# Duy1230/Map-Reduced-Approach-for-Vietnamese-Long-Document-Summarization

Hardware: AMD Instinct MI355X
Metric: map-phase chunks/sec (2k-tok chunk, 256-tok summary) at 1/2/4/8 MI355X (higher is better)
Workload: dtype f16

## Files before the change

map-reduced-approach-for-vietnamese-long-document-summarization_amd/csrc/gemv_common.h:

```cpp
#pragma once
#include "kernels.h"

namespace ms {

__device__ __forceinline__ uint4 ldg16(const void* p) { return *(const uint4*)p; }

__device__ __forceinline__ uint4 ldw16(const void* p) { return *(const uint4*)p; }

__host__ __device__ constexpr int vmcnt_imm(int n) { return (n & 0xF) | ((n >> 4) << 14) | (0x7 << 4) | (0xF << 8); }

__device__ __forceinline__ void lds_sync() {
  __builtin_amdgcn_fence(__ATOMIC_RELEASE, "workgroup", "local");
  __builtin_amdgcn_s_barrier();
  __builtin_amdgcn_fence(__ATOMIC_ACQUIRE, "workgroup", "local");
}

__host__ __device__ inline size_t gemv_x_lds_bytes(int M, int K) {
  return ((size_t)M * K * 2 + 1023) / 1024 * 1024;
}
__device__ __forceinline__ int x_lds(int r, int k, int K) { return r * 2 * K + (((k >> 3) ^ (r & 7)) << 4); }

__device__ __forceinline__ void gemv_dma_x(char* smem, const f16_t* __restrict__ X, int M, int K, int ldx) {
  const int kch = K >> 3, n = M * kch, lane = threadIdx.x & 63, nw = blockDim.x >> 6;
  for (int p = threadIdx.x >> 6; p * 64 < n; p += nw) {
    const int P = min(p * 64 + lane, n - 1);
    const int r = P / kch, c = P - r * kch;
    __builtin_amdgcn_global_load_lds((const void*)(X + (size_t)r * ldx + ((c ^ (r & 7)) << 3)),
                                     (LDS_AS void*)(smem + (size_t)p * 1024), 16, 0, 0);
  }
}

__host__ __device__ inline size_t gemv_xw_lds_bytes(int M, int K) { return (size_t)((M + 7) >> 3) * K * 16; }
__device__ __forceinline__ int xw_swz(int r) {
  const int t = r >> 1;
  return ((((t >> 1) ^ (t >> 2)) & 1) << 2) | ((t & 1) << 1) | ((t >> 2) & 1);
}
__device__ __forceinline__ int xw_lds(int r, int u, int c, int mp) {
  return (u * mp * 8 + r) * 128 + ((c ^ xw_swz(r)) << 4);
}
template <int U>
__device__ __forceinline__ void gemv_dma_x_wave(char* smem, const f16_t* __restrict__ X, int M, int ldx,
                                                int kbeg) {
  const int lane = threadIdx.x & 63, wave = threadIdx.x >> 6, mp = (M + 7) >> 3;
  char* base = smem + (size_t)wave * U * mp * 1024;
#pragma unroll 1
  for (int j = 0; j < mp; ++j) {
    const int r = j * 8 + (lane >> 3);
    const f16_t* src = X + (size_t)min(r, M - 1) * ldx + kbeg + (((lane & 7) ^ xw_swz(r)) << 3);
#pragma unroll
    for (int u = 0; u < U; ++u)
      __builtin_amdgcn_global_load_lds((const void*)(src + u * 64), (LDS_AS void*)(base + (size_t)(u * mp + j) * 1024),
                                       16, 0, 0);
  }
}

enum { kXGlobal = 0, kXLds = 1, kXRegs = 2, kXWave = 3 };

constexpr int kRsStage = 4096;
__host__ __device__ inline int rs_stage_floats(const RowScale& rs, int M) {
  const int n = rs.tiles * M;
  return (rs.ssq && n <= kRsStage) ? (n + 63) / 64 * 64 : 0;
}
__host__ __device__ inline size_t gemv_rinv_offset(size_t main_bytes) { return (main_bytes + 15) / 16 * 16; }
__host__ __device__ inline size_t gemv_lds_total(size_t main_bytes, const RowScale& rs, int M) {
  return gemv_rinv_offset(main_bytes) + 64 * 4 + (size_t)rs_stage_floats(rs, M) * 4;
}
template <bool HOLD>
__device__ __forceinline__ float rs_begin(char* smem, size_t rinv_off, const RowScale& rs, int M) {
  const int lane = threadIdx.x & 63, wave = threadIdx.x >> 6, nw = blockDim.x >> 6;
  if constexpr (HOLD)
    if (rs.tiles == 1) return (wave == 0 && lane < M) ? rs.ssq[lane] : 0.f;
  const int nf = rs_stage_floats(rs, M), n = rs.tiles * M;
  float* stage = (float*)(smem + rinv_off) + 64;
  for (int p = wave; p * 64 < nf; p += nw)
    __builtin_amdgcn_global_load_lds((const void*)(rs.ssq + min(p * 64 + lane, n - 1)),
                                     (LDS_AS void*)(stage + p * 64), 4, 0, 0);
  return 0.f;
}
template <bool HOLD>
__device__ __forceinline__ void rs_finish(const char* smem, size_t rinv_off, const RowScale& rs, int M,
                                          float direct) {
  const int lane = threadIdx.x & 63, wave = threadIdx.x >> 6, nw = blockDim.x >> 6;
  float* rinv = (float*)(smem + rinv_off);
  if (HOLD && rs.tiles == 1) {
    if (wave == 0 && lane < M) rinv[lane] = rs_rinv(direct, rs);
    return;
  }
  const float* stage = rinv + 64;
  for (int row = wave; row < M; row += nw) {
    float sum = 0.f;
    for (int t = lane; t < ((rs.tiles + 63) & ~63); t += 64) sum += t < rs.tiles ? stage[t * M + row] : 0.f;
    sum = wave_sum(sum);
    if (lane == 0) rinv[row] = rs_rinv(sum, rs);
  }
}

template <int EPI> constexpr bool gemv_rs_epi() {
  return EPI == MS_GEMV_EPI_STORE_F16 || EPI == MS_GEMV_EPI_SWIGLU || EPI == MS_GEMV_EPI_STORE_F32 ||
         EPI == MS_GEMV_EPI_ROPE_KV;
}

constexpr int kXRegsMaxFrags = 4;
enum { kGxLds = 0, kGxRegs = 1, kGxF32 = 2, kGxResid = 3, kGxBoth = 4 };
inline int gemv_x_mode() {
  static const int v = [] {
    const char* e = getenv("MS_GEMV_X");
    if (!e) return kGxLds;
    const char c = e[0];
    return c == 'r' && e[1] == 'e' && e[2] == 'g' ? kGxRegs : c == 'f' ? kGxF32 : c == 'r' ? kGxResid
         : c == 'b' ? kGxBoth : kGxLds;
  }();
  return v;
}
inline bool gemv_x_regs_for(int epi) {
  const int m = gemv_x_mode();
  const bool f32 = epi == MS_GEMV_EPI_STORE_F32, resid = epi == MS_GEMV_EPI_RESID_SSQ;
  return m == kGxRegs || ((m == kGxF32 || m == kGxBoth) && f32) || ((m == kGxResid || m == kGxBoth) && resid);
}
inline int qgemv_x_mode() {
  static const int v = [] {
    const char* e = getenv("MS_QGEMV_X");
    if (!e) return 2;
    return e[0] == 'r' ? 0 : e[0] == 'l' ? 1 : e[0] == 'g' ? 2 : e[0] == 's' ? 3 : 2;
  }();
  return v;
}

__device__ __forceinline__ void amax_merge_dev(float& v, int& i, float v2, int i2) {
  if (v2 > v || (v2 == v && i2 < i)) { v = v2; i = i2; }
}

struct ResidPre {
  float x, g;
};
template <int MT, int NT, int EPI, bool RS>
__device__ __forceinline__ void gemv_epilogue(const float* red, const float* rinv, int M, int N, int ldo,
                                              void* __restrict__ out, int n0, const GemvArgs& ga,
                                              const ResidPre& pre);
__device__ __forceinline__ void gemv_elem(int e, int NT, int n0, int& row, int& col, int& c) {
  const int mn = e >> 8, l = (e >> 2) & 63, j = e & 3;
  row = (mn / NT) * 16 + 4 * (l >> 4) + j;
  c = l & 15;
  col = n0 + (mn % NT) * 16 + c;
}
template <int EPI, bool RAW = false>
__device__ __forceinline__ ResidPre resid_prefetch(int M, int N, int ldo, const void* out, int n0,
                                                   const GemvArgs& ga) {
  ResidPre p{0.f, 0.f};
  if constexpr (EPI == MS_GEMV_EPI_RESID_SSQ) {
    const int rtv = ga.rt > 0 ? ga.rt : 16;
    if ((int)threadIdx.x < 256) {
      int row, col, c;
      gemv_elem(threadIdx.x, 1, n0, row, col, c);
      if (row < M && c < rtv && col < N) {
        p.x = ((const float*)out)[(size_t)row * ldo + col];
        if (ga.xg_out) p.g = RAW ? __uint_as_float((unsigned)ga.gamma[col]) : h2f(ga.gamma[col]);
      }
    }
  }
  return p;
// ... 143 lines not shown
```

map-reduced-approach-for-vietnamese-long-document-summarization_amd/csrc/k_gemv.hip:

```cpp
#include "gemv_common.h"

namespace ms {

struct GemvPlan {
  int MT, NT, waves, U, tiles;
};

static GemvPlan gemv_plan(int M, int N, int K, int epi, int force_waves = 0, int rt = 0) {
  GemvPlan p;
  p.MT = (M + 15) / 16;
  p.NT = (epi == MS_GEMV_EPI_SWIGLU) ? 2 : 1;
  const int rows = p.NT == 1 && rt > 0 ? rt : 16 * p.NT;
  p.tiles = (N + rows - 1) / rows;
  const int steps = K / 64;
  int best_w = 0;
  if (force_waves > 0 && steps % force_waves == 0 && steps / force_waves <= 8) {
    best_w = force_waves;
  } else {
    for (int w = 16; w >= 1; --w)
      if (steps % w == 0 && steps / w <= 8) { best_w = w; break; }
  }
  p.waves = best_w;
  p.U = best_w ? steps / best_w : 0;
  return p;
}

size_t gemv_workspace_bytes(int, int, int) { return 256; }

constexpr size_t kMaxLds = 160 * 1024;

static size_t gemv_lds_main(const GemvPlan& p, int M, int K, int xm) {
  size_t xs = xm == kXLds ? gemv_x_lds_bytes(M, K) : xm == kXWave ? gemv_xw_lds_bytes(M, K) : 0;
  const size_t red = (size_t)p.waves * p.MT * p.NT * 256 * 4;
  return xs > red ? xs : red;
}
static size_t gemv_lds_bytes(const GemvPlan& p, int M, int K, int xm, const RowScale& rs = RowScale{}) {
  return gemv_lds_total(gemv_lds_main(p, M, K, xm), rs, M);
}

constexpr int kGvStampBlocks = 1024, kGvStamps = 32;
__device__ unsigned long long g_gemv_stamps[kGvStampBlocks * kGvStamps];
#define GV_STAMP(k)                                     \
  do {                                                  \
    if constexpr (STAMP) {                              \
      __builtin_amdgcn_sched_barrier(0);                \
      ts[k] = __builtin_amdgcn_s_memrealtime();         \
      __builtin_amdgcn_sched_barrier(0);                \
    }                                                   \
  } while (0)

template <int MT, int NT, int EPI, int U, int XM, bool RS, bool WF, bool STAMP>
__device__ __forceinline__ void gemv_body(const f16_t* __restrict__ X, const f16_t* __restrict__ W,
                                          void* __restrict__ out, int M, int N, int K, int ldk, int ldo,
                                          int rinv_off, const GemvArgs& ga) {
  static_assert(!WF || XM == kXLds || XM == kXWave, "weight-first applies to the DMA-staged forms");
  static_assert(XM != kXWave || WF, "per-wave slices come with the weight-first order");
  extern __shared__ __attribute__((aligned(16))) char smem[];
  const int tid = threadIdx.x, lane = tid & 63, wave = tid >> 6;
  const int fr = lane & 15, fg = lane >> 4;
  unsigned long long ts[STAMP ? 12 : 1] = {};
  GV_STAMP(0);
  const int rt = NT == 1 && ga.rt > 0 ? ga.rt : 16;
  const int n0 = blockIdx.x * (NT == 1 ? rt : 16 * NT);
  const int kbeg = wave * U * 64;
  if constexpr (EPI == MS_GEMV_EPI_STORE_F32) {
    X += (size_t)blockIdx.y * K;
    W += (size_t)blockIdx.y * K;
    out = (float*)out + (size_t)blockIdx.y * (ga.slab_rows > 0 ? ga.slab_rows : M) * ldo;
  }
  constexpr bool kXL = XM == kXLds || XM == kXWave;
  constexpr bool kRsEarly = kXL && NT == 1;
  constexpr bool kBar = XM == kXLds || (RS && NT == 1);
  constexpr int kAfterX = WF ? (U - 1) * NT * 2 : U * NT * 2;

  uint4 w[U][NT][2];
  if constexpr (WF) {
#pragma unroll
    for (int n = 0; n < NT; ++n) {
      const int wrow = NT == 1 ? n0 + min(fr, rt - 1) : n0 + n * 16 + fr;
      const f16_t* wp = W + (size_t)min(wrow, N - 1) * ldk + kbeg + 16 * fg;
      w[0][n][0] = ldw16(wp);
      w[0][n][1] = ldw16(wp + 8);
    }
    GV_STAMP(2);
    __builtin_amdgcn_sched_barrier(0);
  }
  if constexpr (RS) rs_begin<false>(smem, rinv_off, ga.rs, M);
  ResidPre pre = resid_prefetch<EPI, WF>(M, N, ldo, out, n0, ga);
  if constexpr (XM == kXLds) gemv_dma_x(smem, X, M, K, ldk);
  if constexpr (XM == kXWave) gemv_dma_x_wave<U>(smem, X, M, ldk, kbeg);
  uint4 xr[XM == kXRegs ? U : 1][XM == kXRegs ? MT : 1][2];
  if constexpr (XM == kXRegs) {
#pragma unroll
    for (int u = 0; u < U; ++u)
#pragma unroll
      for (int m = 0; m < MT; ++m) {
        const f16_t* xg = X + (size_t)min(m * 16 + fr, M - 1) * ldk + kbeg + u * 64 + 16 * fg;
        xr[u][m][0] = ldg16(xg);
        xr[u][m][1] = ldg16(xg + 8);
      }
  }
  GV_STAMP(3);
  __builtin_amdgcn_sched_barrier(0);
  if constexpr (WF) {
#pragma unroll
    for (int u = 1; u < U; ++u)
#pragma unroll
      for (int n = 0; n < NT; ++n) {
        const int wrow = NT == 1 ? n0 + min(fr, rt - 1) : n0 + n * 16 + fr;
        const f16_t* wp = W + (size_t)min(wrow, N - 1) * ldk + kbeg + 16 * fg;
        w[u][n][0] = ldw16(wp + u * 64);
        w[u][n][1] = ldw16(wp + u * 64 + 8);
      }
  } else {
#pragma unroll
    for (int n = 0; n < NT; ++n) {
      const int wrow = NT == 1 ? n0 + min(fr, rt - 1) : n0 + n * 16 + fr;
      const f16_t* wp = W + (size_t)min(wrow, N - 1) * ldk + kbeg + 16 * fg;
#pragma unroll
      for (int u = 0; u < U; ++u) {
        w[u][n][0] = ldw16(wp + u * 64);
        w[u][n][1] = ldw16(wp + u * 64 + 8);
        if (n == 0 && u == 0) GV_STAMP(2);
      }
    }
  }
  GV_STAMP(4);
  if constexpr (kXL) {
    __builtin_amdgcn_sched_barrier(0);
    __builtin_amdgcn_s_waitcnt(vmcnt_imm(kAfterX));
    GV_STAMP(5);
    if constexpr (kBar) __builtin_amdgcn_s_barrier();
    GV_STAMP(6);
    if constexpr (RS && NT == 1) rs_finish<false>(smem, rinv_off, ga.rs, M, 0.f);
  }

  f32x4 acc[MT][NT];
#pragma unroll
  for (int m = 0; m < MT; ++m)
#pragma unroll
    for (int n = 0; n < NT; ++n) acc[m][n] = f32x4{0.f, 0.f, 0.f, 0.f};
  const int mp = (M + 7) >> 3;
  const char* xw = smem + (size_t)wave * U * mp * 1024;
#pragma unroll
  for (int u = 0; u < U; ++u) {
    if constexpr (STAMP) {
      if (u == 0) {
        __builtin_amdgcn_s_waitcnt(vmcnt_imm(WF ? (U - 1) * NT * 2 : (U - 1) * 2));
        GV_STAMP(7);
      }
      if (u == U - 1) {
        __builtin_amdgcn_s_waitcnt(vmcnt_imm(0));
        GV_STAMP(8);
      }
    }
#pragma unroll
    for (int m = 0; m < MT; ++m) {
      const int xrow = min(m * 16 + fr, M - 1);
      f16x8 x0, x1;
      if constexpr (XM == kXRegs) {
        x0 = as_f16x8(xr[u][m][0]);
        x1 = as_f16x8(xr[u][m][1]);
      } else if constexpr (XM == kXLds) {
        const int k0 = kbeg + u * 64 + 16 * fg;
        x0 = *(const f16x8*)(smem + x_lds(xrow, k0, K));
        x1 = *(const f16x8*)(smem + x_lds(xrow, k0 + 8, K));
      } else if constexpr (XM == kXWave) {
        x0 = *(const f16x8*)(xw + xw_lds(xrow, u, 2 * fg, mp));
        x1 = *(const f16x8*)(xw + xw_lds(xrow, u, 2 * fg + 1, mp));
      } else {
        const f16_t* xg = X + (size_t)xrow * ldk + kbeg + u * 64 + 16 * fg;
        x0 = as_f16x8(ldg16(xg));
        x1 = as_f16x8(ldg16(xg + 8));
      }
#pragma unroll
      for (int n = 0; n < NT; ++n) {
        acc[m][n] = mfma16(x0, as_f16x8(w[u][n][0]), acc[m][n]);
        acc[m][n] = mfma16(x1, as_f16x8(w[u][n][1]), acc[m][n]);
      }
    }
  }
  if constexpr (WF && EPI == MS_GEMV_EPI_RESID_SSQ) resid_gain(pre);
  GV_STAMP(9);
  unsigned long long* t_red = nullptr;
  if constexpr (STAMP) t_red = &ts[10];
  gemv_finish<MT, NT, EPI, RS, kRsEarly, false>(acc, smem, rinv_off, M, N, ldo, out, n0, ga, pre, 0.f, t_red);
  if constexpr (STAMP) {
    GV_STAMP(11);
    const int nw = blockDim.x >> 6, blk = blockIdx.y * gridDim.x + blockIdx.x;
    if (lane == 0 && (wave == 0 || wave == nw - 1) && blk < kGvStampBlocks) {
      unsigned hw, xcc;
      asm volatile("s_getreg_b32 %0, hwreg(HW_REG_HW_ID)" : "=s"(hw));
      asm volatile("s_getreg_b32 %0, hwreg(HW_REG_XCC_ID)" : "=s"(xcc));
      ts[1] = ((unsigned long long)xcc << 32) | hw;
      unsigned long long* dst = g_gemv_stamps + (size_t)blk * kGvStamps + (wave == 0 ? 0 : 16);
#pragma unroll
      for (int k = 0; k < 12; ++k) dst[k] = ts[k];
    }
  }
}

template <int MT, int NT, int EPI, int U, int XM, bool RS>
__global__ __launch_bounds__(1024) void gemv_kernel(const f16_t* __restrict__ X,
                                                    const f16_t* __restrict__ W,
                                                    void* __restrict__ out, int M, int N, int K,
                                                    int ldk, int ldo, int rinv_off, GemvArgs ga) {
  extern __shared__ __attribute__((aligned(16))) char smem[];
  const int tid = threadIdx.x, lane = tid & 63, wave = tid >> 6;
  const int fr = lane & 15, fg = lane >> 4;
  const int rt = NT == 1 && ga.rt > 0 ? ga.rt : 16;
  const int n0 = blockIdx.x * (NT == 1 ? rt : 16 * NT);
  const int kbeg = wave * U * 64;
  if constexpr (EPI == MS_GEMV_EPI_STORE_F32) {
    X += (size_t)blockIdx.y * K;
    W += (size_t)blockIdx.y * K;
    out = (float*)out + (size_t)blockIdx.y * (ga.slab_rows > 0 ? ga.slab_rows : M) * ldo;
  }

  constexpr bool kRsEarly = XM == kXLds && NT == 1;
  if constexpr (RS) rs_begin<false>(smem, rinv_off, ga.rs, M);
  const ResidPre pre = resid_prefetch<EPI>(M, N, ldo, out, n0, ga);
  if constexpr (XM == kXLds) gemv_dma_x(smem, X, M, K, ldk);
  uint4 xr[XM == kXRegs ? U : 1][XM == kXRegs ? MT : 1][2];
  if constexpr (XM == kXRegs) {
#pragma unroll
    for (int u = 0; u < U; ++u)
#pragma unroll
      for (int m = 0; m < MT; ++m) {
        const f16_t* xg = X + (size_t)min(m * 16 + fr, M - 1) * ldk + kbeg + u * 64 + 16 * fg;
        xr[u][m][0] = ldg16(xg);
        xr[u][m][1] = ldg16(xg + 8);
      }
  }
  __builtin_amdgcn_sched_barrier(0);
  uint4 w[U][NT][2];
#pragma unroll
  for (int n = 0; n < NT; ++n) {
    const int wrow = NT == 1 ? n0 + min(fr, rt - 1) : n0 + n * 16 + fr;
    const f16_t* wp = W + (size_t)min(wrow, N - 1) * ldk + kbeg + 16 * fg;
#pragma unroll
    for (int u = 0; u < U; ++u) {
      w[u][n][0] = ldw16(wp + u * 64);
      w[u][n][1] = ldw16(wp + u * 64 + 8);
    }
  }
  if constexpr (XM == kXLds) {
    __builtin_amdgcn_sched_barrier(0);
    __builtin_amdgcn_s_waitcnt(vmcnt_imm(U * NT * 2));
    __builtin_amdgcn_s_barrier();
    if constexpr (RS && NT == 1) rs_finish<false>(smem, rinv_off, ga.rs, M, 0.f);
  }

  f32x4 acc[MT][NT];
#pragma unroll
  for (int m = 0; m < MT; ++m)
#pragma unroll
    for (int n = 0; n < NT; ++n) acc[m][n] = f32x4{0.f, 0.f, 0.f, 0.f};
#pragma unroll
  for (int u = 0; u < U; ++u) {
#pragma unroll
    for (int m = 0; m < MT; ++m) {
      const int xrow = min(m * 16 + fr, M - 1);
      f16x8 x0, x1;
      if constexpr (XM == kXRegs) {
        x0 = as_f16x8(xr[u][m][0]);
        x1 = as_f16x8(xr[u][m][1]);
      } else if constexpr (XM == kXLds) {
        const int k0 = kbeg + u * 64 + 16 * fg;
        x0 = *(const f16x8*)(smem + x_lds(xrow, k0, K));
        x1 = *(const f16x8*)(smem + x_lds(xrow, k0 + 8, K));
      } else {
        const f16_t* xg = X + (size_t)xrow * ldk + kbeg + u * 64 + 16 * fg;
        x0 = as_f16x8(ldg16(xg));
        x1 = as_f16x8(ldg16(xg + 8));
      }
#pragma unroll
      for (int n = 0; n < NT; ++n) {
        acc[m][n] = mfma16(x0, as_f16x8(w[u][n][0]), acc[m][n]);
        acc[m][n] = mfma16(x1, as_f16x8(w[u][n][1]), acc[m][n]);
      }
    }
  }
  gemv_finish<MT, NT, EPI, RS, kRsEarly, false>(acc, smem, rinv_off, M, N, ldo, out, n0, ga, pre);
}

template <int MT, int NT, int EPI, int U, int XM, bool RS>
__global__ __launch_bounds__(1024) void gemv_wf_kernel(const f16_t* __restrict__ X,
                                                       const f16_t* __restrict__ W,
                                                       void* __restrict__ out, int M, int N, int K,
                                                       int ldk, int ldo, int rinv_off, GemvArgs ga) {
  gemv_body<MT, NT, EPI, U, XM, RS, true, false>(X, W, out, M, N, K, ldk, ldo, rinv_off, ga);
}

template <int NT, int EPI, int U, int XM, bool RS, bool WF>
__global__ __launch_bounds__(1024) void gemv_stamp_kernel(const f16_t* __restrict__ X,
                                                          const f16_t* __restrict__ W,
                                                          void* __restrict__ out, int M, int N, int K,
                                                          int ldk, int ldo, int rinv_off, GemvArgs ga) {
  gemv_body<1, NT, EPI, U, XM, RS, WF, true>(X, W, out, M, N, K, ldk, ldo, rinv_off, ga);
}

void gemv_stamps(unsigned long long* host, int n) {
  n = std::min(n, kGvStampBlocks * kGvStamps);
  (void)hipMemcpyFromSymbol(host, HIP_SYMBOL(g_gemv_stamps), (size_t)n * sizeof(unsigned long long));
  void* p = nullptr;
  if (hipGetSymbolAddress(&p, HIP_SYMBOL(g_gemv_stamps)) == hipSuccess)
    (void)hipMemset(p, 0, sizeof(unsigned long long) * kGvStampBlocks * kGvStamps);
}

static bool gemv_stamps_on() {
  static const bool on = [] { const char* e = getenv("MS_GEMV_STAMPS"); return e && atoi(e); }();
  return on;
}

enum { kGcQkv = 0, kGcO, kGcGateUp, kGcDown, kGcLmHead, kGcCount };
static int g_gemv_class_order[kGcCount] = {0, 2, 1, 2, 0};
static int g_gemv_order = [] {
  const char* e = getenv("MS_GEMV_ORDER");
  if (!e || !e[0]) return -1;
  auto dig = [](char c) { return c >= '0' && c <= '2' ? c - '0' : 0; };
  if (!e[1]) return dig(e[0]);
  for (int i = 0; i < kGcCount && e[i]; ++i) g_gemv_class_order[i] = dig(e[i]);
  return -1;
}();
void set_gemv_order(int v) { g_gemv_order = v; }
static int gemv_order_for(int epi, int N, int U) {
  if (g_gemv_order >= 0) return g_gemv_order;
  if (epi == MS_GEMV_EPI_SWIGLU) return g_gemv_class_order[kGcGateUp];
  if (epi == MS_GEMV_EPI_RESID_SSQ) return g_gemv_class_order[U <= 4 ? kGcO : kGcDown];
  if (epi == MS_GEMV_EPI_ARGMAX || (epi == MS_GEMV_EPI_STORE_F32 && N >= 65536)) return g_gemv_class_order[kGcLmHead];
  if (epi == MS_GEMV_EPI_STORE_F32) return g_gemv_class_order[kGcQkv];
  return 0;
}

template <int MT, int NT, int EPI, int U, bool RS>
static void gemv_go_rs(const f16_t* X, const f16_t* W, void* out, int M, int N, int K, int ldk,
                       const dim3& grid, const dim3& blk, size_t lds, int ro, int ldo, int xm, int ord,
                       const GemvArgs& ga, hipStream_t s) {
#define GL(...) MS_LAUNCH((__VA_ARGS__), grid, blk, lds, s, X, W, out, M, N, K, ldk, ldo, ro, ga)
  if constexpr (MT * U <= kXRegsMaxFrags) {
    if (xm == kXRegs) {
      GL(gemv_kernel<MT, NT, EPI, U, kXRegs, RS>);
      return;
    }
  }
  constexpr bool kStampEpi = EPI == MS_GEMV_EPI_STORE_F32 || EPI == MS_GEMV_EPI_SWIGLU ||
                             EPI == MS_GEMV_EPI_RESID_SSQ || EPI == MS_GEMV_EPI_ARGMAX;
  if constexpr (MT == 1 && (U == 1 || U == 3 || U == 8) && kStampEpi) {
    if (gemv_stamps_on() && (xm == kXLds || xm == kXWave)) {
      if (xm == kXWave) GL(gemv_stamp_kernel<NT, EPI, U, kXWave, RS, true>);
      else if (ord) GL(gemv_stamp_kernel<NT, EPI, U, kXLds, RS, true>);
      else GL(gemv_stamp_kernel<NT, EPI, U, kXLds, RS, false>);
      return;
    }
  }
  if (xm == kXWave) GL(gemv_wf_kernel<MT, NT, EPI, U, kXWave, RS>);
  else if (xm == kXLds && ord) GL(gemv_wf_kernel<MT, NT, EPI, U, kXLds, RS>);
  else if (xm == kXLds) GL(gemv_kernel<MT, NT, EPI, U, kXLds, RS>);
  else GL(gemv_kernel<MT, NT, EPI, U, kXGlobal, RS>);
#undef GL
}

template <int MT, int NT, int EPI, int U>
static void gemv_go(const f16_t* X, const f16_t* W, void* out, int M, int N, int K, int ldk,
                    int S, int ldo, const GemvPlan& p, size_t lds, int xm, int ord, const GemvArgs& ga,
                    hipStream_t s) {
  const dim3 grid(p.tiles, S), blk(64 * p.waves);
  const int ro = (int)gemv_rinv_offset(gemv_lds_main(p, M, K, xm));
  if constexpr (EPI == MS_GEMV_EPI_ROPE_KV && MT != 1) {
    return;
  } else if constexpr (gemv_rs_epi<EPI>()) {
    if (ga.rs.ssq) gemv_go_rs<MT, NT, EPI, U, true>(X, W, out, M, N, K, ldk, grid, blk, lds, ro, ldo, xm, ord, ga, s);
    else gemv_go_rs<MT, NT, EPI, U, false>(X, W, out, M, N, K, ldk, grid, blk, lds, ro, ldo, xm, ord, ga, s);
  } else {
    gemv_go_rs<MT, NT, EPI, U, false>(X, W, out, M, N, K, ldk, grid, blk, lds, ro, ldo, xm, ord, ga, s);
  }
}

template <int MT, int NT, int EPI>
static void gemv_go_u(const f16_t* X, const f16_t* W, void* out, int M, int N, int K, int ldk,
                      int S, int ldo, const GemvPlan& p, size_t lds, int xm, int ord, const GemvArgs& ga,
                      hipStream_t s) {
#define GU(U_) gemv_go<MT, NT, EPI, U_>(X, W, out, M, N, K, ldk, S, ldo, p, lds, xm, ord, ga, s)
  switch (p.U) {
    case 1: GU(1); break;
    case 2: GU(2); break;
    case 3: GU(3); break;
    case 4: GU(4); break;
    case 5: GU(5); break;
    case 6: GU(6); break;
    case 7: GU(7); break;
    default: GU(8); break;
  }
#undef GU
}

template <int MT>
static void gemv_go_mt(const f16_t* X, const f16_t* W, void* out, int M, int N, int K, int ldk,
                       int S, int ldo, int epi, const GemvPlan& p, size_t lds, int xm, int ord,
                       const GemvArgs& ga, hipStream_t s) {
#define GE(NT_, E_) gemv_go_u<MT, NT_, E_>(X, W, out, M, N, K, ldk, S, ldo, p, lds, xm, ord, ga, s)
  switch (epi) {
    case MS_GEMV_EPI_STORE_F16: GE(1, MS_GEMV_EPI_STORE_F16); break;
    case MS_GEMV_EPI_ADD_F32: GE(1, MS_GEMV_EPI_ADD_F32); break;
    case MS_GEMV_EPI_SWIGLU: GE(2, MS_GEMV_EPI_SWIGLU); break;
    case MS_GEMV_EPI_ROPE_KV: GE(1, MS_GEMV_EPI_ROPE_KV); break;
    case MS_GEMV_EPI_ARGMAX: GE(1, MS_GEMV_EPI_ARGMAX); break;
    case MS_GEMV_EPI_RESID_SSQ: GE(1, MS_GEMV_EPI_RESID_SSQ); break;
    default: GE(1, MS_GEMV_EPI_STORE_F32); break;
  }
#undef GE
}

bool gemv_supported(int M, int N, int K, int epi, int rs_tiles) {
  if (M < 1 || M > 64 || K % 64) return false;
  if (epi == MS_GEMV_EPI_ROPE_KV && M > 16) return false;
  if (epi == MS_GEMV_EPI_ARGMAX && N % 16) return false;
  const GemvPlan p = gemv_plan(M, N, K, epi);
  if (p.waves == 0) return false;
  if (epi == MS_GEMV_EPI_RESID_SSQ && p.waves < 4) return false;
  if (epi == MS_GEMV_EPI_ROPE_KV && gemv_lds_bytes(p, M, K, kXLds) > kMaxLds) return false;
  RowScale rs{};
  const bool takes_rs = epi != MS_GEMV_EPI_ARGMAX && epi != MS_GEMV_EPI_ADD_F32 && epi != MS_GEMV_EPI_RESID_SSQ;
  if (rs_tiles > 0 && takes_rs) {
    if (!gemv_rs_supported(M, rs_tiles)) return false;
    rs = make_row_scale(reinterpret_cast<const float*>(16), rs_tiles, 1, 0.f);
  }
  return gemv_lds_bytes(p, M, K, kXGlobal, rs) <= kMaxLds;
}

static void gemv_dispatch(const f16_t* X, const f16_t* W, void* out, int M, int N, int K, int ldk,
                          int S, int ldo, int epi, const GemvArgs* ga_in, int force_waves,
                          hipStream_t s) {
  if (M <= 0) return;
  const int rt = ga_in ? ga_in->rt : 0;
  const GemvPlan p = gemv_plan(M, N, K, epi, force_waves, rt);
  if (p.waves == 0) return;
  GemvArgs ga{};
  if (ga_in) ga = *ga_in;
  if (epi == MS_GEMV_EPI_ARGMAX || epi == MS_GEMV_EPI_ADD_F32 || epi == MS_GEMV_EPI_RESID_SSQ)
    ga.rs = RowScale{};
  const bool xl = gemv_lds_bytes(p, M, K, kXLds, ga.rs) <= kMaxLds;
  int xm = xl ? kXLds : kXGlobal;
  const int ord = xl ? gemv_order_for(epi, N, p.U) : 0;
  if (ord == 2 && gemv_lds_bytes(p, M, K, kXWave, ga.rs) <= kMaxLds) xm = kXWave;
  if (gemv_x_regs_for(epi) && p.MT * p.U <= kXRegsMaxFrags) xm = kXRegs;
  if (ga.rs.ssq && rs_stage_floats(ga.rs, M) == 0) return;
  const size_t lds = gemv_lds_bytes(p, M, K, xm, ga.rs);
  if (lds > kMaxLds) return;
  switch (p.MT) {
    case 1: gemv_go_mt<1>(X, W, out, M, N, K, ldk, S, ldo, epi, p, lds, xm, ord, ga, s); break;
    case 2: gemv_go_mt<2>(X, W, out, M, N, K, ldk, S, ldo, epi, p, lds, xm, ord, ga, s); break;
    case 3: gemv_go_mt<3>(X, W, out, M, N, K, ldk, S, ldo, epi, p, lds, xm, ord, ga, s); break;
    default: gemv_go_mt<4>(X, W, out, M, N, K, ldk, S, ldo, epi, p, lds, xm, ord, ga, s); break;
  }
}

void launch_gemv_ex(const f16_t* X, const f16_t* W, void* out, int M, int N, int K, int ldo,
                    int epi, const GemvArgs* ga_in, int force_waves, hipStream_t s) {
  gemv_dispatch(X, W, out, M, N, K, K, 1, ldo, epi, ga_in, force_waves, s);
}

void launch_gemv_strided(const f16_t* X, const f16_t* W, void* out, int M, int N, int K, int ldk,
                         int ldo, int epi, hipStream_t s) {
  gemv_dispatch(X, W, out, M, N, K, ldk, 1, ldo, epi, nullptr, 0, s);
}

bool gemv_rs_supported(int M, int tiles) { return M >= 1 && tiles >= 1 && tiles * M <= kRsStage; }

bool gemv_split_supported(int M, int N, int K, int S, int rs_tiles) {
  if (S < 1 || K % S) return false;
  return gemv_supported(M, N, K / S, MS_GEMV_EPI_STORE_F32, rs_tiles);
}

void launch_gemv_split(const f16_t* X, const f16_t* W, float* slabs, int M, int N, int K, int S,
                       int force_waves, hipStream_t s, const GemvArgs* ga) {
  gemv_dispatch(X, W, slabs, M, N, K / S, K, S, N, MS_GEMV_EPI_STORE_F32, ga, force_waves, s);
}

__global__ __launch_bounds__(1024) void argmax_partials_kernel(const float2* __restrict__ part, int tiles,
                                                               int32_t* __restrict__ out) {
  __shared__ float sv[16];
  __shared__ int si[16];
  const float2* p = part + (size_t)blockIdx.x * tiles;
  float v = -INFINITY;
  int idx = 0x7FFFFFFF;
  for (int t0 = 0; t0 < tiles; t0 += 8 * 1024) {
    float2 q[8];
#pragma unroll
    for (int i = 0; i < 8; ++i) {
      const int t = t0 + i * 1024 + threadIdx.x;
      q[i] = t < tiles ? p[t] : make_float2(-INFINITY, __int_as_float(0x7FFFFFFF));
    }
#pragma unroll
    for (int i = 0; i < 8; ++i) amax_merge_dev(v, idx, q[i].x, __float_as_int(q[i].y));
  }
#pragma unroll
  for (int o = 32; o > 0; o >>= 1) amax_merge_dev(v, idx, __shfl_xor(v, o, 64), __shfl_xor(idx, o, 64));
  if ((threadIdx.x & 63) == 0) { sv[threadIdx.x >> 6] = v; si[threadIdx.x >> 6] = idx; }
  __syncthreads();
  if (threadIdx.x == 0) {
    for (int w = 1; w < 16; ++w) amax_merge_dev(v, idx, sv[w], si[w]);
    out[blockIdx.x] = (idx == 0x7FFFFFFF || !__builtin_isfinite(v)) ? -1 : idx;
  }
}

void launch_argmax_partials(const void* partials, int rows, int tiles, int32_t* out, hipStream_t s) {
  if (rows <= 0) return;
  MS_LAUNCH(argmax_partials_kernel, dim3(rows), dim3(1024), 0, s, (const float2*)partials, tiles, out);
}

void launch_gemv(const f16_t* X, const f16_t* W, void* out, int M, int N, int K, int ldo, int epi,
                 void*, hipStream_t s) {
  launch_gemv_ex(X, W, out, M, N, K, ldo, epi, nullptr, 0, s);
}

}
```

map-reduced-approach-for-vietnamese-long-document-summarization_amd/csrc/ops.cpp:

```cpp
#include <cstdint>
#include <functional>

#include "internal.h"
#include "kernels.h"

using namespace ms;

static int op_guard(const std::function<void()>& fn) {
  try {
    fn();
    hipError_t err = hipGetLastError();
    if (err != hipSuccess) {
      g_last_error = std::string("kernel launch failed: ") + hipGetErrorString(err);
      return MS_EIO;
    }
    return MS_OK;
  } catch (const MsError& x) {
    g_last_error = x.what();
    return x.code;
  }
}

template <class Fn>
static int checked(bool ok, Fn&& fn) {
  if (!ok) return MS_EINVAL;
  fn();
  return MS_OK;
}

static thread_local RowScale g_op_rs{};
static int op_rs_tiles() { return g_op_rs.ssq ? g_op_rs.tiles : 0; }

static const GemvArgs* op_gemv_args(GemvArgs& ga) {
  ga = GemvArgs{};
  ga.rs = g_op_rs;
  return g_op_rs.ssq ? &ga : nullptr;
}

static GemvArgs op_resid_args(int rt, float* ssq_out, const void* gamma, void* xg_out) {
  GemvArgs ga{};
  ga.rt = rt;
  ga.ssq_out = ssq_out;
  ga.gamma = (const f16_t*)gamma;
  ga.xg_out = (f16_t*)xg_out;
  return ga;
}

static QMat op_qmat(int type, const void* packed, int K) {
  QMat q{};
  q.n = 1;
  q.base0 = (const uint8_t*)packed;
  q.row0_0 = 0;
  q.type0 = type;
  q.row_bytes0 = (K / 256) * qblock_bytes(type, true);
  return q;
}

extern "C" {

int ms_op_set_row_scale(const float* ssq, int32_t tiles, int32_t hidden, float eps) {
  if (ssq && (tiles < 1 || hidden < 1)) return MS_EINVAL;
  g_op_rs = ssq ? make_row_scale(ssq, tiles, hidden, eps) : RowScale{};
  return MS_OK;
}

int ms_op_gemm(const void* A, const void* W, void* out, int32_t M, int32_t N, int32_t K, int32_t ldo,
               int32_t epi, void* stream) {
  return op_guard([&] {
    REQUIRE(A && W && out && M >= 1 && N >= 16 && K >= 64 && K % 64 == 0, MS_EINVAL, "bad gemm shape");
    REQUIRE(((epi >= 0 && epi <= 3) || epi == MS_EPI_ARGMAX) && (epi != MS_EPI_SWIGLU || N % 32 == 0), MS_EINVAL,
            "bad epilogue");
    REQUIRE(epi != MS_EPI_ADD_F32 || (N % 4 == 0 && ldo % 4 == 0), MS_EINVAL,
            "residual gemm: N and ldo multiples of 4 (16-B x rows)");
    REQUIRE(epi != MS_EPI_ARGMAX || (N % 16 == 0 && ldo >= N / 16), MS_EINVAL, "gemm argmax: N % 16, ldo >= N / 16");
    REQUIRE(((uintptr_t)out & ((epi == MS_EPI_ADD_F32 || epi == MS_EPI_STORE_F32) ? 15 : 7)) == 0, MS_EINVAL,
            "gemm: out must be 16-B (fp32) / 8-B (fp16) aligned");
    REQUIRE(!g_op_rs.ssq || gemm_rs_tiles_ok(M, N, g_op_rs.tiles), MS_EINVAL,
            "gemm row scale: at most 24 tiles of statistics (kGemmRsTiles, both GEMM tiles)");
    launch_gemm((const f16_t*)A, (const f16_t*)W, out, M, N, K, ldo, epi == MS_EPI_ARGMAX ? MS_GEMV_EPI_ARGMAX : epi,
                (hipStream_t)stream, &g_op_rs);
  });
}

int ms_op_gemm_resid(const void* A, const void* W, float* x, void* xg_out, const void* gamma, float* ssq_out,
                     int32_t M, int32_t N, int32_t K, void* stream) {
  return op_guard([&] {
    REQUIRE(A && W && x && xg_out && gamma && ssq_out && M >= 1 && N >= 16 && K >= 64 && K % 64 == 0, MS_EINVAL,
            "bad gemm_resid operands (K % 64 == 0)");
    REQUIRE(gemm_resid_tiles(M, N) <= kGemmRsTiles, MS_EINVAL, "gemm_resid: N over 24 column tiles");
    REQUIRE(N % 4 == 0 && ((uintptr_t)x & 15) == 0 && ((uintptr_t)xg_out & 7) == 0, MS_EINVAL,
            "gemm_resid: N a multiple of 4, x 16-B and xg 8-B aligned (vector rows)");
    GemmResid gr{(const f16_t*)gamma, (f16_t*)xg_out, ssq_out};
    launch_gemm((const f16_t*)A, (const f16_t*)W, x, M, N, K, N, MS_EPI_ADD_F32, (hipStream_t)stream, nullptr, &gr);
  });
}

int ms_gemm_resid_tiles(int32_t M, int32_t N) { return gemm_resid_tiles(M, N); }

int ms_set_gemm_variant(int32_t v) { return checked(v >= 0 && v <= 4, [&] { set_gemm_variant(v); }); }
int ms_set_gemv_order(int32_t order) { return checked(order >= -1 && order <= 2, [&] { set_gemv_order(order); }); }
int ms_set_attn_tuning(int32_t combine_grp, int32_t order) {
  return checked(combine_grp >= 0 && combine_grp <= 1 && (order == 0 || order == 3),
                 [&] { set_attn_tuning(combine_grp, order); });
}
int ms_set_dgemm_kh(int32_t kh) { return checked(kh == 1 || kh == 2, [&] { set_dgemm_kh(kh); }); }
int ms_set_dgemm_wn(int32_t wn) { return checked(wn == 4 || wn == 8, [&] { set_dgemm_wn(wn); }); }
int ms_set_qgemv_gs(int32_t on) { return checked(on >= 0 && on <= 1, [&] { set_qgemv_gs(on != 0); }); }

static int stamps(void (*read)(unsigned long long*, int), uint64_t* out, int32_t n) {
  return checked(out && n >= 0, [&] { read(reinterpret_cast<unsigned long long*>(out), n); });
}
int ms_debug_gemv_stamps(uint64_t* out, int32_t n) { return stamps(gemv_stamps, out, n); }
int ms_debug_pk_stamps(uint64_t* out, int32_t n) { return stamps(persist_stamps, out, n); }
int ms_debug_a2_stamps(uint64_t* out, int32_t n) { return stamps(attn2_stamps, out, n); }

int64_t ms_op_gemv_workspace(int32_t M, int32_t N, int32_t K) {
  if (M < 1 || M > 64 || N < 16 || K < 64 || K % 64) return MS_EINVAL;
  return (int64_t)gemv_workspace_bytes(M, N, K);
}

int ms_op_gemv(const void* X, const void* W, void* out, int32_t M, int32_t N, int32_t K, int32_t ldo,
               int32_t epi, void* ws, void* stream) {
  return ms_op_gemv_tuned(X, W, out, M, N, K, ldo, epi, ws, 0, stream);
}

int ms_op_gemv_tuned(const void* X, const void* W, void* out, int32_t M, int32_t N, int32_t K,
                     int32_t ldo, int32_t epi, void* ws, int32_t waves, void* stream) {
  return op_guard([&] {
    REQUIRE(X && W && out && ws && N >= 16 && N % 16 == 0, MS_EINVAL, "bad gemv operands");
    REQUIRE(((epi >= 0 && epi <= 3) || epi == MS_EPI_ARGMAX) && (epi != MS_EPI_SWIGLU || N % 32 == 0),
            MS_EINVAL, "bad epilogue");
    REQUIRE(gemv_supported(M, N, K, epi, op_rs_tiles()), MS_EINVAL,
            "gemv shape unsupported (M<=64, K%64==0, K/64 split into <=16 waves of <=8 steps; "
            "row-scale statistics within kRsStage and LDS)");
    GemvArgs ga;
    launch_gemv_ex((const f16_t*)X, (const f16_t*)W, out, M, N, K, ldo, epi, op_gemv_args(ga), waves,
                   (hipStream_t)stream);
  });
}

int ms_op_gemv_strided(const void* X, const void* W, void* out, int32_t M, int32_t N, int32_t K,
                       int32_t ldk, int32_t ldo, int32_t epi, void* stream) {
  return op_guard([&] {
    REQUIRE(X && W && out && N >= 16 && N % 16 == 0 && ldk >= K && ldk % 8 == 0, MS_EINVAL,
            "bad strided gemv operands");
    REQUIRE(epi >= 0 && epi <= 3 && epi != MS_EPI_SWIGLU, MS_EINVAL, "bad epilogue");
    REQUIRE(gemv_supported(M, N, K, epi), MS_EINVAL, "gemv shape unsupported");
    launch_gemv_strided((const f16_t*)X, (const f16_t*)W, out, M, N, K, ldk, ldo, epi, (hipStream_t)stream);
  });
}

int ms_op_gemv_resid(const void* X, const void* W, float* x, void* xg_out, const void* gamma,
                     float* ssq_out, int32_t M, int32_t N, int32_t K, int32_t rt, void* stream) {
  return op_guard([&] {
    REQUIRE(X && W && x && xg_out && gamma && ssq_out && rt >= 1 && rt <= 16 && N >= 1, MS_EINVAL,
            "bad gemv_resid operands");
    REQUIRE(gemv_supported(M, N, K, MS_GEMV_EPI_RESID_SSQ), MS_EINVAL, "gemv_resid shape unsupported");
    const GemvArgs ga = op_resid_args(rt, ssq_out, gamma, xg_out);
    launch_gemv_ex((const f16_t*)X, (const f16_t*)W, x, M, N, K, N, MS_GEMV_EPI_RESID_SSQ, &ga, 0,
                   (hipStream_t)stream);
  });
}

int ms_op_dgemm(const void* X, const void* W, void* out, int32_t M, int32_t N, int32_t K, int32_t S,
                int32_t ldo, int32_t epi, void* stream) {
  return op_guard([&] {
    REQUIRE(X && W && out, MS_EINVAL, "bad dgemm operands");
    REQUIRE(((epi >= 0 && epi <= 3) || epi == MS_EPI_ARGMAX) && dgemm_supported(M, N, K, S, epi), MS_EINVAL,
            "dgemm shape unsupported (M <= 256, N % 64 == 0, K % (64 S) == 0, S > 1 only for fp32 slabs)");
    REQUIRE(!g_op_rs.ssq || g_op_rs.tiles == 1, MS_EINVAL, "dgemm row scale: one-tile statistics only");
    launch_dgemm((const f16_t*)X, (const f16_t*)W, out, M, N, K, S, ldo, epi, (hipStream_t)stream, &g_op_rs);
  });
}

int ms_op_gemv_split(const void* X, const void* W, float* slabs, int32_t M, int32_t N, int32_t K,
                     int32_t S, int32_t waves, void* stream) {
  return op_guard([&] {
    REQUIRE(X && W && slabs && N >= 16 && S >= 1, MS_EINVAL, "bad gemv_split operands");
    REQUIRE(gemv_split_supported(M, N, K, S, op_rs_tiles()), MS_EINVAL,
            "gemv_split shape unsupported (M<=64, (K/S)%64==0, row-scale statistics within kRsStage and LDS)");
    GemvArgs ga;
    launch_gemv_split((const f16_t*)X, (const f16_t*)W, slabs, M, N, K, S, waves, (hipStream_t)stream,
                      op_gemv_args(ga));
  });
}

int ms_op_residual_rmsnorm(float* x, const float* slabs, int32_t S, const void* w, void* y, float* ssq,
                           int32_t rows, int32_t hidden, void* stream) {
  return op_guard([&] {
    REQUIRE(x && w && y && ssq && rows >= 1 && hidden >= 4 && hidden % 4 == 0 && hidden <= 8192, MS_EINVAL,
            "bad residual_rmsnorm shape");
    REQUIRE(S == 0 || slabs, MS_EINVAL, "slabs missing");
    REQUIRE(residual_rmsnorm_supported(S, hidden) || (S == 0 && hidden <= 8192), MS_EINVAL,
            "residual_rmsnorm: S <= 8 and hidden <= 3072 (wider rows: S == 0 only)");
    launch_residual_rmsnorm(x, slabs, S, (const f16_t*)w, (f16_t*)y, ssq, rows, hidden,
                            (hipStream_t)stream);
  });
}

int ms_op_dequant(int32_t type, const void* blocks, int64_t n_blocks, float* out, void* stream) {
  return op_guard([&] {
    REQUIRE(blocks && out && n_blocks >= 1, MS_EINVAL, "bad dequant arguments");
    REQUIRE(qtype_known(type), MS_EINVAL, "ggml type must be Q8_0, Q4_K, Q5_K or Q6_K");
    launch_dequant_f32(type, (const uint8_t*)blocks, n_blocks, out, (hipStream_t)stream);
  });
}

int ms_op_quant_rows(int32_t type, const void* blocks, int32_t rows, int32_t K, void* f16_out,
                     void* packed_out, void* stream) {
  return op_guard([&] {
    REQUIRE(blocks && f16_out && rows >= 1 && K >= 256 && K % 256 == 0, MS_EINVAL, "bad quant_rows arguments");
    REQUIRE(qtype_known(type), MS_EINVAL, "ggml type must be Q8_0, Q4_K, Q5_K or Q6_K");
    launch_quant_rows(type, (const uint8_t*)blocks, rows, K, (f16_t*)f16_out, 16, 0,
                      (uint8_t*)packed_out, 0, (hipStream_t)stream);
  });
}

int ms_op_qgemv(const void* X, int32_t type, const void* packed, void* out, int32_t M, int32_t N,
                int32_t K, int32_t ldo, int32_t epi, void* stream) {
  return op_guard([&] {
    REQUIRE(X && packed && out && N >= 16, MS_EINVAL, "bad qgemv operands");
    REQUIRE(qtype_known(type), MS_EINVAL, "ggml type must be Q8_0, Q4_K, Q5_K or Q6_K");
    REQUIRE(((epi >= 0 && epi <= 3) || epi == MS_EPI_ARGMAX) && (epi != MS_EPI_SWIGLU || N % 32 == 0),
            MS_EINVAL, "bad epilogue");
    REQUIRE(qgemv_supported(M, N, K, epi, op_rs_tiles()), MS_EINVAL,
            "qgemv shape unsupported (M<=64, K%256==0, N%16==0, row-scale statistics within kRsStage and LDS)");
    GemvArgs ga;
    launch_qgemv((const f16_t*)X, op_qmat(type, packed, K), out, M, N, K, ldo, epi, op_gemv_args(ga),
                 (hipStream_t)stream);
  });
}

int ms_op_qgemv_split(const void* X, int32_t type, const void* packed, float* slabs, int32_t M,
                      int32_t N, int32_t K, int32_t S, void* stream) {
  return op_guard([&] {
    REQUIRE(X && packed && slabs && N >= 16 && S >= 1, MS_EINVAL, "bad qgemv_split operands");
    REQUIRE(qtype_known(type), MS_EINVAL, "ggml type must be Q8_0, Q4_K, Q5_K or Q6_K");
    REQUIRE(qgemv_split_supported(M, N, K, S, op_rs_tiles()), MS_EINVAL,
            "qgemv_split shape unsupported (M<=64, K%(256*S)==0, row-scale statistics within kRsStage and LDS)");
    GemvArgs ga;
    launch_qgemv_split((const f16_t*)X, op_qmat(type, packed, K), slabs, M, N, K, S, (hipStream_t)stream,
                       op_gemv_args(ga));
  });
}

int ms_op_qgemv_resid(const void* X, int32_t type, const void* packed, float* x, void* xg_out, const void* gamma,
                      float* ssq_out, int32_t M, int32_t N, int32_t K, int32_t rt, void* stream) {
  return op_guard([&] {
    REQUIRE(X && packed && x && xg_out && gamma && ssq_out && rt >= 1 && rt <= 16 && N % rt == 0, MS_EINVAL,
            "bad qgemv_resid operands");
    REQUIRE(qtype_known(type), MS_EINVAL, "ggml type must be Q8_0, Q4_K, Q5_K or Q6_K");
    REQUIRE(qgemv_supported(M, N, K, MS_GEMV_EPI_RESID_SSQ), MS_EINVAL, "qgemv_resid shape unsupported");
    const GemvArgs ga = op_resid_args(rt, ssq_out, gamma, xg_out);
    launch_qgemv((const f16_t*)X, op_qmat(type, packed, K), x, M, N, K, N, MS_GEMV_EPI_RESID_SSQ, &ga,
                 (hipStream_t)stream);
  });
}

int ms_op_qdgemm(const void* X, int32_t type, const void* packed, void* out, int32_t M, int32_t N, int32_t K,
                 int32_t S, int32_t ldo, int32_t epi, void* stream) {
  return op_guard([&] {
    REQUIRE(X && packed && out && N >= 64 && K >= 256 && S >= 1, MS_EINVAL, "bad qdgemm operands");
    REQUIRE(type != MS_QT_Q8_0, MS_EINVAL,
            "qdgemm has no Q8_0 form (Q8_0 engines run their fp16 copies in the large regime): Q4_K, Q5_K, Q6_K or F16");
    REQUIRE(type == MS_QT_Q4_K || type == MS_QT_Q5_K || type == MS_QT_Q6_K || type == 1, MS_EINVAL,
            "ggml type must be Q4_K, Q5_K, Q6_K or F16");
    REQUIRE(!g_op_rs.ssq || g_op_rs.tiles == 1, MS_EINVAL, "qdgemm row scale: one-tile statistics only");
    const int e = epi == MS_EPI_ARGMAX ? MS_GEMV_EPI_ARGMAX : epi;
    if (type == 1) {
      REQUIRE(qdgemm_f16_supported(M, N, K, S, e), MS_EINVAL, "qdgemm (fp16 rows) shape unsupported");
      launch_qdgemm_f16((const f16_t*)X, (const f16_t*)packed, out, M, N, K, S, ldo, e, (hipStream_t)stream, &g_op_rs);
      return;
    }
    const QMat q = op_qmat(type, packed, K);
    REQUIRE(qdgemm_supported(M, N, K, S, e, q), MS_EINVAL,
            "qdgemm shape unsupported (M <= 256, N % 64 == 0, K % (256 S) == 0, S > 1 only for fp32 slabs)");
    launch_qdgemm((const f16_t*)X, q, out, M, N, K, S, ldo, e, (hipStream_t)stream, &g_op_rs);
  });
}

int ms_op_rmsnorm(const void* x, const void* w, void* y, float* ssq, int32_t rows, int32_t hidden,
                  const int32_t* row_idx, void* stream) {
// ... 58 lines not shown
```

Measured before the change: 12.98.

## Add lane-exchange weight load layout with nontemporal loads to GEMV

Adds a GEMV variant in which each lane loads a contiguous 16-byte weight chunk whose addressing covers 8 rows by 2 halves. A DPP row-shift exchange afterwards restores the per-lane fragment layout the MFMA expects, which is meant to give more coalesced global weight reads. A further mode issues these loads as nontemporal so streamed weights do not pollute cache. The default per-class order now selects order 8 (LX=2 with the wave-sliced X form) for the O, gate/up, down and LM-head GEMVs. The cost is extra DPP instructions and scheduling barriers per step, plus one more kernel instantiation per shape. Ragged N is also now allowed for store epilogues.

New measurement: 13.17 (median of 6 runs). +1.5%, better.

```diff
diff --git a/map-reduced-approach-for-vietnamese-long-document-summarization_amd/csrc/gemv_common.h b/map-reduced-approach-for-vietnamese-long-document-summarization_amd/csrc/gemv_common.h
--- a/map-reduced-approach-for-vietnamese-long-document-summarization_amd/csrc/gemv_common.h
+++ b/map-reduced-approach-for-vietnamese-long-document-summarization_amd/csrc/gemv_common.h
@@ -6,6 +6,24 @@
 __device__ __forceinline__ uint4 ldg16(const void* p) { return *(const uint4*)p; }
 
 __device__ __forceinline__ uint4 ldw16(const void* p) { return *(const uint4*)p; }
+__device__ __forceinline__ uint4 ldw16_nt(const void* p) {
+  typedef unsigned u32x4 __attribute__((ext_vector_type(4)));
+  const u32x4 v = __builtin_nontemporal_load((const u32x4*)p);
+  return make_uint4(v.x, v.y, v.z, v.w);
+}
+
+__device__ __forceinline__ void lx_exchange(uint4& a, uint4& b, bool hi) {
+  auto swap = [&](unsigned& A, unsigned& B) {
+    const int send = (int)(hi ? A : B);
+    const unsigned recv = (unsigned)__builtin_amdgcn_update_dpp(send, send, 0x128 , 0xF, 0xF, false);
+    A = hi ? recv : A;
+    B = hi ? B : recv;
+  };
+  swap(a.x, b.x);
+  swap(a.y, b.y);
+  swap(a.z, b.z);
+  swap(a.w, b.w);
+}
 
 __host__ __device__ constexpr int vmcnt_imm(int n) { return (n & 0xF) | ((n >> 4) << 14) | (0x7 << 4) | (0xF << 8); }
 
diff --git a/map-reduced-approach-for-vietnamese-long-document-summarization_amd/csrc/k_gemv.hip b/map-reduced-approach-for-vietnamese-long-document-summarization_amd/csrc/k_gemv.hip
--- a/map-reduced-approach-for-vietnamese-long-document-summarization_amd/csrc/k_gemv.hip
+++ b/map-reduced-approach-for-vietnamese-long-document-summarization_amd/csrc/k_gemv.hip
@@ -49,7 +49,7 @@
     }                                                   \
   } while (0)
 
-template <int MT, int NT, int EPI, int U, int XM, bool RS, bool WF, bool STAMP>
+template <int MT, int NT, int EPI, int U, int XM, bool RS, bool WF, bool STAMP, int LX = 0>
 __device__ __forceinline__ void gemv_body(const f16_t* __restrict__ X, const f16_t* __restrict__ W,
                                           void* __restrict__ out, int M, int N, int K, int ldk, int ldo,
                                           int rinv_off, const GemvArgs& ga) {
@@ -74,13 +74,25 @@
   constexpr int kAfterX = WF ? (U - 1) * NT * 2 : U * NT * 2;
 
   uint4 w[U][NT][2];
+  auto wrow_lx = [&](int n, int half) {
+    const int r = (fr & 7) + half;
+    const int wrow = NT == 1 ? n0 + min(r, rt - 1) : n0 + n * 16 + r;
+    const unsigned off = (unsigned)((min(wrow, N - 1) - n0) * ldk + kbeg + 16 * fg + 8 * (fr >> 3)) * 2u;
+    return (const f16_t*)((const char*)(W + (size_t)n0 * ldk) + off);
+  };
+  auto ldw = [](const f16_t* p) { return LX == 2 ? ldw16_nt(p) : ldw16(p); };
   if constexpr (WF) {
 #pragma unroll
     for (int n = 0; n < NT; ++n) {
-      const int wrow = NT == 1 ? n0 + min(fr, rt - 1) : n0 + n * 16 + fr;
-      const f16_t* wp = W + (size_t)min(wrow, N - 1) * ldk + kbeg + 16 * fg;
-      w[0][n][0] = ldw16(wp);
-      w[0][n][1] = ldw16(wp + 8);
+      if constexpr (LX) {
+        w[0][n][0] = ldw(wrow_lx(n, 0));
+        w[0][n][1] = ldw(wrow_lx(n, 8));
+      } else {
+        const int wrow = NT == 1 ? n0 + min(fr, rt - 1) : n0 + n * 16 + fr;
+        const f16_t* wp = W + (size_t)min(wrow, N - 1) * ldk + kbeg + 16 * fg;
+        w[0][n][0] = ldw16(wp);
+        w[0][n][1] = ldw16(wp + 8);
+      }
     }
     GV_STAMP(2);
     __builtin_amdgcn_sched_barrier(0);
@@ -107,20 +119,26 @@
     for (int u = 1; u < U; ++u)
 #pragma unroll
       for (int n = 0; n < NT; ++n) {
-        const int wrow = NT == 1 ? n0 + min(fr, rt - 1) : n0 + n * 16 + fr;
-        const f16_t* wp = W + (size_t)min(wrow, N - 1) * ldk + kbeg + 16 * fg;
-        w[u][n][0] = ldw16(wp + u * 64);
-        w[u][n][1] = ldw16(wp + u * 64 + 8);
+        if constexpr (LX) {
+          w[u][n][0] = ldw(wrow_lx(n, 0) + u * 64);
+          w[u][n][1] = ldw(wrow_lx(n, 8) + u * 64);
+        } else {
+          const int wrow = NT == 1 ? n0 + min(fr, rt - 1) : n0 + n * 16 + fr;
+          const f16_t* wp = W + (size_t)min(wrow, N - 1) * ldk + kbeg + 16 * fg;
+          w[u][n][0] = ldw16(wp + u * 64);
+          w[u][n][1] = ldw16(wp + u * 64 + 8);
+        }
       }
   } else {
 #pragma unroll
     for (int n = 0; n < NT; ++n) {
       const int wrow = NT == 1 ? n0 + min(fr, rt - 1) : n0 + n * 16 + fr;
-      const f16_t* wp = W + (size_t)min(wrow, N - 1) * ldk + kbeg + 16 * fg;
+      const f16_t* wp = LX ? wrow_lx(n, 0) : W + (size_t)min(wrow, N - 1) * ldk + kbeg + 16 * fg;
+      const f16_t* wq = LX ? wrow_lx(n, 8) : wp + 8;
 #pragma unroll
       for (int u = 0; u < U; ++u) {
-        w[u][n][0] = ldw16(wp + u * 64);
-        w[u][n][1] = ldw16(wp + u * 64 + 8);
+        w[u][n][0] = ldw(wp + u * 64);
+        w[u][n][1] = ldw(wq + u * 64);
         if (n == 0 && u == 0) GV_STAMP(2);
       }
     }
@@ -133,6 +151,7 @@
     if constexpr (kBar) __builtin_amdgcn_s_barrier();
     GV_STAMP(6);
     if constexpr (RS && NT == 1) rs_finish<false>(smem, rinv_off, ga.rs, M, 0.f);
+    if constexpr (LX) __builtin_amdgcn_sched_barrier(0);
   }
 
   f32x4 acc[MT][NT];
@@ -153,6 +172,11 @@
         __builtin_amdgcn_s_waitcnt(vmcnt_imm(0));
         GV_STAMP(8);
       }
+    }
+    if constexpr (LX) {
+#pragma unroll
+      for (int n = 0; n < NT; ++n) lx_exchange(w[u][n][0], w[u][n][1], fr >> 3);
+      if constexpr (NT == 2) __builtin_amdgcn_sched_barrier(0);
     }
 #pragma unroll
     for (int m = 0; m < MT; ++m) {
@@ -292,6 +316,14 @@
   gemv_body<MT, NT, EPI, U, XM, RS, true, false>(X, W, out, M, N, K, ldk, ldo, rinv_off, ga);
 }
 
+template <int MT, int NT, int EPI, int U, int XM, bool RS, bool WF, int LX>
+__global__ __launch_bounds__(1024) void gemv_lx_kernel(const f16_t* __restrict__ X,
+                                                       const f16_t* __restrict__ W,
+                                                       void* __restrict__ out, int M, int N, int K,
+                                                       int ldk, int ldo, int rinv_off, GemvArgs ga) {
+  gemv_body<MT, NT, EPI, U, XM, RS, WF, false, LX>(X, W, out, M, N, K, ldk, ldo, rinv_off, ga);
+}
+
 template <int NT, int EPI, int U, int XM, bool RS, bool WF>
 __global__ __launch_bounds__(1024) void gemv_stamp_kernel(const f16_t* __restrict__ X,
                                                           const f16_t* __restrict__ W,
@@ -313,12 +345,13 @@
   return on;
 }
 
+constexpr int kGemvOrders = 9;
 enum { kGcQkv = 0, kGcO, kGcGateUp, kGcDown, kGcLmHead, kGcCount };
-static int g_gemv_class_order[kGcCount] = {0, 2, 1, 2, 0};
+static int g_gemv_class_order[kGcCount] = {0, 8, 8, 8, 8};
 static int g_gemv_order = [] {
   const char* e = getenv("MS_GEMV_ORDER");
   if (!e || !e[0]) return -1;
-  auto dig = [](char c) { return c >= '0' && c <= '2' ? c - '0' : 0; };
+  auto dig = [](char c) { return c >= '0' && c < '0' + kGemvOrders ? c - '0' : 0; };
   if (!e[1]) return dig(e[0]);
   for (int i = 0; i < kGcCount && e[i]; ++i) g_gemv_class_order[i] = dig(e[i]);
   return -1;
@@ -335,9 +368,23 @@
 
 template <int MT, int NT, int EPI, int U, bool RS>
 static void gemv_go_rs(const f16_t* X, const f16_t* W, void* out, int M, int N, int K, int ldk,
-                       const dim3& grid, const dim3& blk, size_t lds, int ro, int ldo, int xm, int ord,
+                       const dim3& grid, const dim3& blk, size_t lds, int ro, int ldo, int xm, int sel,
                        const GemvArgs& ga, hipStream_t s) {
+  const int ord = sel % 3, lx = sel / 3;
 #define GL(...) MS_LAUNCH((__VA_ARGS__), grid, blk, lds, s, X, W, out, M, N, K, ldk, ldo, ro, ga)
+  if constexpr (MT == 1)
+  if (lx && !gemv_stamps_on() && (xm == kXLds || xm == kXWave)) {
+#define GLX(LX_)                                                                     \
+  do {                                                                                 \
+    if (xm == kXWave) GL(gemv_lx_kernel<MT, NT, EPI, U, kXWave, RS, true, LX_>);        \
+    else if (ord) GL(gemv_lx_kernel<MT, NT, EPI, U, kXLds, RS, true, LX_>);             \
+    else GL(gemv_lx_kernel<MT, NT, EPI, U, kXLds, RS, false, LX_>);                     \
+  } while (0)
+    if (lx == 1) GLX(1);
+    else GLX(2);
+#undef GLX
+    return;
+  }
   if constexpr (MT * U <= kXRegsMaxFrags) {
     if (xm == kXRegs) {
       GL(gemv_kernel<MT, NT, EPI, U, kXRegs, RS>);
@@ -443,7 +490,7 @@
   const bool xl = gemv_lds_bytes(p, M, K, kXLds, ga.rs) <= kMaxLds;
   int xm = xl ? kXLds : kXGlobal;
   const int ord = xl ? gemv_order_for(epi, N, p.U) : 0;
-  if (ord == 2 && gemv_lds_bytes(p, M, K, kXWave, ga.rs) <= kMaxLds) xm = kXWave;
+  if (ord % 3 == 2 && gemv_lds_bytes(p, M, K, kXWave, ga.rs) <= kMaxLds) xm = kXWave;
   if (gemv_x_regs_for(epi) && p.MT * p.U <= kXRegsMaxFrags) xm = kXRegs;
   if (ga.rs.ssq && rs_stage_floats(ga.rs, M) == 0) return;
   const size_t lds = gemv_lds_bytes(p, M, K, xm, ga.rs);
diff --git a/map-reduced-approach-for-vietnamese-long-document-summarization_amd/csrc/ops.cpp b/map-reduced-approach-for-vietnamese-long-document-summarization_amd/csrc/ops.cpp
--- a/map-reduced-approach-for-vietnamese-long-document-summarization_amd/csrc/ops.cpp
+++ b/map-reduced-approach-for-vietnamese-long-document-summarization_amd/csrc/ops.cpp
@@ -98,7 +98,7 @@
 int ms_gemm_resid_tiles(int32_t M, int32_t N) { return gemm_resid_tiles(M, N); }
 
 int ms_set_gemm_variant(int32_t v) { return checked(v >= 0 && v <= 4, [&] { set_gemm_variant(v); }); }
-int ms_set_gemv_order(int32_t order) { return checked(order >= -1 && order <= 2, [&] { set_gemv_order(order); }); }
+int ms_set_gemv_order(int32_t order) { return checked(order >= -1 && order <= 8, [&] { set_gemv_order(order); }); }
 int ms_set_attn_tuning(int32_t combine_grp, int32_t order) {
   return checked(combine_grp >= 0 && combine_grp <= 1 && (order == 0 || order == 3),
                  [&] { set_attn_tuning(combine_grp, order); });
@@ -127,7 +127,8 @@
 int ms_op_gemv_tuned(const void* X, const void* W, void* out, int32_t M, int32_t N, int32_t K,
                      int32_t ldo, int32_t epi, void* ws, int32_t waves, void* stream) {
   return op_guard([&] {
-    REQUIRE(X && W && out && ws && N >= 16 && N % 16 == 0, MS_EINVAL, "bad gemv operands");
+    const bool ragged_ok = epi == MS_EPI_STORE_F16 || epi == MS_EPI_STORE_F32;
+    REQUIRE(X && W && out && ws && N >= 16 && (N % 16 == 0 || ragged_ok), MS_EINVAL, "bad gemv operands");
     REQUIRE(((epi >= 0 && epi <= 3) || epi == MS_EPI_ARGMAX) && (epi != MS_EPI_SWIGLU || N % 32 == 0),
             MS_EINVAL, "bad epilogue");
     REQUIRE(gemv_supported(M, N, K, epi, op_rs_tiles()), MS_EINVAL,
```
